# chengl7-lab/scape

Measured on AMD Instinct MI355X. Metric: UTR regions/sec (infer_pa EM to convergence), 50k UTRs x 2k reads synthetic, higher is better.
Workload: dtype f64; 1 GPU; 50k-UTR synthetic stream x 2000 reads, K=1..10 x 10 restarts; step = one resident batch of 512 UTRs per GPU; reads_per_utr=2000, k_cap=10, n_frag_max=1469, re_run_mode=False, rng_mode=per_utr, parallelism=utr-shard x1

## Files before the change

scape_amd/csrc/em_lockstep.inc:

```

#define MT_RB 1
#define MT_ROWS (64 * MT_RB)
#define MT_NC 32
#define MT_PITCH (MT_NC + 2)
#define MT_VPITCH (MT_NC + 2)
#define MT_MAXJ 64
#ifndef EM_DEPTH
#define EM_DEPTH 3
#endif
static_assert(EM_DEPTH >= 1 && EM_DEPTH <= 8, "column slots per job");
#ifndef MT_DV1
#define MT_DV1 1
#endif

#ifndef MT_DEEP
#define MT_DEEP 2
#endif
#define CNT_DONE 3
#define CNT_SLAB 4
#define CNT_EXEC (4 + 64)
#define CNT_MSTEP_TENSOR (4 + 2 * 64)
#define CNT_MSTEP_VREQ (4 + 3 * 64)
#define CNT_MSTEP_VUNI (4 + 4 * 64)
static_assert(MT_ROWS == TILE_ROWS, "tile height must match k_tile_extent / the host tables");
static_assert(MT_MAXJ <= 64, "the per-pass job setup gives one job to each lane of one wavefront");

struct EmState {
    int32_t *ia, *ib, *sia, *sib;
    double *ws, *slw;
    double *lb, *ell;
    int32_t *nlb, *status;
    unsigned long long *pend;
    int32_t *rd_k, *rd_lo, *rd_hi, *rd_m;
    int32_t *rd_n0, *rd_n1;
    double *rd_lw, *rd_sv;
    double *rd_fl;
    double *V;
    double *Vsuf;
    const int64_t *voff;
    double *pt_score;
    int32_t *pt_row;
    const int64_t *ptoff;
    int32_t *u_done;
};

__device__ __forceinline__ double d_wave_allsum(double v) {
#pragma unroll
    for (int off = 32; off > 0; off >>= 1) v += __shfl_xor(v, off, 64);
    return v;
}

#ifndef ESTEP_EXP_GROUP
#define ESTEP_EXP_GROUP 1
#endif
struct EstepNext {
    int status;
    int nlb;
    int pub_k;
    int k_next;
};

template <int CA, int CX, int NW = 1>
__device__ __forceinline__ EstepNext estep_body(
    const UtrDesc *__restrict__ descs, const DevParams &P, const double *__restrict__ cnt,
    const double *__restrict__ M, int kmax, const int32_t *__restrict__ job_utr,
    const int32_t *__restrict__ job_K, const int32_t *__restrict__ job_fixed,
    const int32_t *__restrict__ a_in, const int32_t *__restrict__ b_in,
    const double *__restrict__ ws_in, const int8_t *__restrict__ k_arr, const EmState &S,
    int32_t *__restrict__ a_out, int32_t *__restrict__ b_out, double *__restrict__ ws_out,
    double *__restrict__ bic_out, int32_t *__restrict__ nlb_out, double *__restrict__ lb_out,
    unsigned long long *__restrict__ counters, int launch, int slot, int depth, int job, int lane, int status,
    unsigned long long *s_roff, double *s_lwc, double *s_wsum ,
    const double2 *s_exptab , int wave = 0, double *s_xz = nullptr ,
    double *s_tot = nullptr ) {
    constexpr int CMAX = CA;
#ifdef ESTEP_STAMPS
    const unsigned long long st0 = __builtin_amdgcn_s_memtime();
#define ESTEP_STAMP(v) const unsigned long long v = __builtin_amdgcn_s_memtime()
#else
#define ESTEP_STAMP(v)
#endif
    const bool lead = (NW == 1) || wave == 0;
    const int nround = P.nround, B = P.B;
    const int u_job = job_utr[job];
    const int K = (CX > 0) ? CX - 1 : job_K[job], C = K + 1;
    const bool fixed = job_fixed[job] != 0;
    int32_t *ia = S.ia + (size_t)job * kmax, *ib = S.ib + (size_t)job * kmax;
    int32_t *sia = S.sia + (size_t)job * kmax, *sib = S.sib + (size_t)job * kmax;
    double *ws = S.ws + (size_t)job * (kmax + 1), *slw = S.slw + (size_t)job * (kmax + 1);
    const bool r0 = launch == 0 && slot == 0;
    const bool resolve = slot == 0 && launch > 0;
    const size_t col0 = (size_t)job * depth, col = col0 + slot;
    int pre_m[EM_DEPTH], pre_lo[EM_DEPTH], pre_hi[EM_DEPTH], pre_k[EM_DEPTH];
    int64_t pre_ptoff[EM_DEPTH];
    double pre_fl[EM_DEPTH];
    bool rdm = false;
#pragma unroll
    for (int q = 0; q < EM_DEPTH; ++q) {
        const bool on = resolve && q < depth;
        pre_m[q] = on ? S.rd_m[col0 + q] : 0;
        pre_lo[q] = on ? S.rd_lo[col0 + q] : 0;
        pre_hi[q] = on ? S.rd_hi[col0 + q] : 0;
        pre_k[q] = on ? S.rd_k[col0 + q] : 0;
        pre_ptoff[q] = on ? S.ptoff[col0 + q] : 0;
        pre_fl[q] = on ? S.rd_fl[col0 + q] : 0.0;
        rdm = rdm || pre_m[q] != 0;
    }
    const int64_t pre_voff = S.voff[col];
    const int k_lane = (lane < nround) ? (int)k_arr[(size_t)job * nround + lane] : 0;
    const double lb_prev = r0 ? SENT : S.lb[job];
    const int nlb_prev = r0 ? 0 : S.nlb[job];
    auto k_of_round = [&](int i) {
        const int ii = min(i, nround - 1);
        return (nround <= 64) ? __shfl(k_lane, ii, 64) : (int)k_arr[(size_t)job * nround + ii];
    };
    const int k_now = k_of_round(nlb_prev);
    const int k_next = __builtin_amdgcn_readfirstlane(k_of_round(nlb_prev + 1));
    double my_ws = 0.0, my_slw = 0.0;
    int my_ia = 0, my_ib = 0, my_sia = 0, my_sib = 0;
    if (lane < C) {
        my_ws = r0 ? ws_in[(size_t)job * (kmax + 1) + lane] : ws[lane];
        if (!r0) my_slw = slw[lane];
        if (lane < K) {
            my_ia = r0 ? a_in[(size_t)job * kmax + lane] : ia[lane];
            my_ib = r0 ? b_in[(size_t)job * kmax + lane] : ib[lane];
            my_sia = r0 ? my_ia : sia[lane];
            my_sib = r0 ? my_ib : sib[lane];
        }
    }
    const UtrDesc d = descs[u_job];
    double pt_best[EM_DEPTH];
    int pt_best_r[EM_DEPTH];
#pragma unroll
    for (int q = 0; q < EM_DEPTH; ++q) {
        pt_best[q] = -INFINITY;
        pt_best_r[q] = pre_lo[q];
        if (pre_m[q]) {
            const int t0 = pre_lo[q] / MT_ROWS, t1 = (pre_hi[q] - 1) / MT_ROWS;
            const double fl = pre_fl[q], ftol = (4.0 * d.Np + 16.0) * 1.1102230246251565e-16 * fabs(fl);
            for (int t = t0 + lane; t <= t1; t += 64) {
                double sc = S.pt_score[pre_ptoff[q] + t];
                const int rr = S.pt_row[pre_ptoff[q] + t];
                if (fabs(sc - fl) <= ftol) sc = fl;
                if (sc > pt_best[q]) {
                    pt_best[q] = sc;
                    pt_best_r[q] = rr;
                }
            }
        }
    }
    const int N = d.N, Np = d.Np;
    const double *Mu = M + (size_t)d.m_off;
    const double *cu = cnt + d.bin_off;
    if (r0) my_slw = d_logw(my_ws);

    if (lead && r0) {
        if (lane < C) {
            ws[lane] = my_ws;
            slw[lane] = my_slw;
            if (lane < K) {
                ia[lane] = sia[lane] = my_ia;
                ib[lane] = sib[lane] = my_ib;
            }
        }
        if (lane == 0) {
            S.lb[job] = SENT;
            S.nlb[job] = 0;
            S.ell[job] = 0.0;
        }
    }
    int upd_k[EM_DEPTH], upd_a[EM_DEPTH], upd_b[EM_DEPTH];
#pragma unroll
    for (int q = 0; q < EM_DEPTH; ++q) {
        upd_k[q] = -1;
        upd_a[q] = upd_b[q] = 0;
        if (pre_m[q]) {
            double best = pt_best[q];
            int best_r = pt_best_r[q];
#pragma unroll
            for (int off = 32; off > 0; off >>= 1) {
                const double ob = __shfl_xor(best, off, 64);
                const int orr = __shfl_xor(best_r, off, 64);
                if (ob > best || (ob == best && orr < best_r)) {
                    best = ob;
                    best_r = orr;
                }
            }
            upd_k[q] = pre_k[q];
            upd_a[q] = best_r / B;
            upd_b[q] = best_r - upd_a[q] * B;
            if (lead && lane == 0) {
                ia[upd_k[q]] = upd_a[q];
                ib[upd_k[q]] = upd_b[q];
            }
            if (lane == upd_k[q]) {
                my_ia = upd_a[q];
                my_ib = upd_b[q];
            }
        }
    }
    if (slot == 0 && lead && lane == 0 && (r0 || rdm))
        for (int q = 0; q < depth; ++q) S.rd_m[col0 + q] = 0;
    auto cur_ia = [&](int i) {
        int v = ia[i];
#pragma unroll
        for (int q = 0; q < EM_DEPTH; ++q) v = (i == upd_k[q]) ? upd_a[q] : v;
        return v;
    };
    auto cur_ib = [&](int i) {
        int v = ib[i];
#pragma unroll
        for (int q = 0; q < EM_DEPTH; ++q) v = (i == upd_k[q]) ? upd_b[q] : v;
        return v;
    };

    if (status == 1 || nlb_prev >= nround) {
        if (lead && lane == 0) {
            const int n_lb = S.nlb[job];
            bic_out[job] = d_bic(S.ell[job], K, N);
            nlb_out[job] = n_lb;
            int idx[CMAX];
            for (int i = 0; i < K; ++i) idx[i] = i;
            for (int i = 1; i < K; ++i) {
                const int v = idx[i];
                int j = i - 1;
                while (j >= 0 && cur_ia(idx[j]) > cur_ia(v)) {
                    idx[j + 1] = idx[j];
                    --j;
                }
                idx[j + 1] = v;
            }
            for (int i = 0; i < K; ++i) {
                a_out[(size_t)job * kmax + i] = cur_ia(idx[i]);
                b_out[(size_t)job * kmax + i] = cur_ib(idx[i]);
                ws_out[(size_t)job * (kmax + 1) + i] = ws[idx[i]];
            }
            ws_out[(size_t)job * (kmax + 1) + K] = ws[K];
            for (int i = K; i < kmax; ++i) {
                a_out[(size_t)job * kmax + i] = -1;
                b_out[(size_t)job * kmax + i] = -1;
                ws_out[(size_t)job * (kmax + 1) + i + 1] = 0.0;
            }
            S.status[job] = 2;
            atomicAdd(&counters[CNT_DONE], 1ull);
            if (S.u_done) atomicAdd(&S.u_done[u_job], 1);
            atomicAdd(&counters[0], (unsigned long long)n_lb);
            atomicAdd(&counters[2], (unsigned long long)n_lb * (unsigned long long)N * (unsigned long long)C);
        }
        return EstepNext{2, nlb_prev, -1, 0};
    }

    if (lead && lane == 0) atomicAdd(&counters[CNT_EXEC + (job & 63)], 1ull);
    const int k = k_now;
    const double wk_old = __shfl(my_ws, k, 64);
    const double slw_k = d_logw(wk_old);
    const int sia_k = (k < K) ? __shfl(my_ia, k, 64) : 0;
    const int sib_k = (k < K) ? __shfl(my_ib, k, 64) : 0;
    const int ia_km1 = __shfl(my_ia, max(k - 1, 0), 64), ia_kp1 = __shfl(my_ia, min(k + 1, 63), 64);
    if (lead && lane == 0) {
        slw[k] = slw_k;
        if (k < K) {
            sia[k] = sia_k;
            sib[k] = sib_k;
        }
    }
    if (lead && lane < CMAX) {
        const int c = lane;
        int sa = 0, sb = 0;
        double lw_c = 0.0;
        if (c < C) {
            if (c == k) {
                lw_c = slw_k;
                sa = sia_k;
                sb = sib_k;
            } else {
                lw_c = my_slw;
                sa = my_sia;
                sb = my_sib;
            }
        }
        s_roff[c] = (c < K) ? ((unsigned long long)sa * B + sb) * Np : 0ull;
        s_lwc[c] = (c < K) ? lw_c : lw_c + d.unif_ll;
    }
    __syncthreads();
    double *Vj = S.V + pre_voff;

    ESTEP_STAMP(st1);
    double tot_w[CMAX], t_sumk = 0.0, t_ell = 0.0, t_ent = 0.0;
    int nz_lo = 0x7fffffff, nz_hi = -1;
    bool mod = false;
    if constexpr (NW == 1) {
        for (int pass = 0; pass < 2; ++pass) {
    #pragma unroll
            for (int c = 0; c < CMAX; ++c) s_wsum[c * 64 + lane] = 0.0;
            double sumk = 0.0, ell = 0.0, ent = 0.0;
            nz_lo = 0x7fffffff;
            nz_hi = -1;
            double mcur[CMAX], ccur = 0.0;
            auto fetch = [&](int n, double (&m)[CMAX], double &cn) {
                const bool ok = n < N;
                cn = ok ? cu[n] : 0.0;
    #pragma unroll
                for (int c = 0; c < CMAX; ++c) m[c] = (ok && c < K) ? Mu[s_roff[c] + n] : 0.0;
            };
            fetch(lane, mcur, ccur);
    #pragma unroll
            for (int c = 0; c < CMAX; ++c) asm volatile("" : "+v"(mcur[c]));
            asm volatile("" : "+v"(ccur));
            for (int n = lane; n < Np; n += 64) {
                double mnext[CMAX], cnext;
                fetch(n + 64, mnext, cnext);
                double vkn = 0.0;
                if (n < N) {
                    const double cn = ccur;
                    auto lzv = [&](int c) { return (c < K) ? s_lwc[c] + mcur[c] : s_lwc[c]; };
                    double mx = 0.0;
    #pragma unroll
                    for (int c = 0; c < CMAX; ++c) {
                        if (c < C) {
                            const double v = lzv(c);
                            mx = (c == 0 || v > mx) ? v : mx;
                        }
                    }
                    double z[CMAX];
                    unsigned long long live = 0ull;
#if ESTEP_EXP_GROUP >= 2
    #pragma unroll
                    for (int c = 0; c < CMAX; c += ESTEP_EXP_GROUP) {
    #pragma unroll
                        for (int i = 0; i < ESTEP_EXP_GROUP; ++i)
                            if (c + i < CMAX) z[c + i] = 0.0;
                        if (c < C) {
                            double arg[ESTEP_EXP_GROUP];
                            bool any_live = false;
    #pragma unroll
                            for (int i = 0; i < ESTEP_EXP_GROUP; ++i) {
                                const bool in = (c + i < CMAX) && (c + i < C);
                                arg[i] = in ? (lzv((c + i < CMAX) ? c + i : c) - mx) * cn : -1000.0;
                                any_live |= arg[i] >= -746.0;
                            }
                            if (__ballot(any_live)) {
    #pragma unroll
                                for (int i = 0; i < ESTEP_EXP_GROUP; ++i)
                                    if (c + i < CMAX)
                                        if (c + i < C) {
                                            live |= 1ull << (c + i);
                                            z[c + i] = d_exp_nonpos(arg[i], s_exptab);
                                        }
                            }
                            __builtin_amdgcn_sched_barrier(0);
                        }
                    }
#else
    #pragma unroll
                    for (int c = 0; c < CMAX; ++c) {
                        z[c] = 0.0;
                        if (c < C) {
                            const double arg = (lzv(c) - mx) * cn;
                            if (__ballot(arg >= -746.0)) {
                                live |= 1ull << c;
                                z[c] = d_exp_nonpos(arg, s_exptab);
                            }
                            __builtin_amdgcn_sched_barrier(0);
                        }
                    }
#endif
                    const double s = d_np_sum<CMAX>(z, C);
                    const double rs = d_rcp_mid(s);
                    double zk = 0.0;
    #pragma unroll
                    for (int c = 0; c < CMAX; ++c) {
                        if (live & (1ull << c)) z[c] = z[c] * rs;
                        if (c == k) {
                            sumk += z[c];
                            if (mod) z[c] += 1e-8;
                            zk = z[c];
                        }
                    }
                    const double s2 = d_np_sum<CMAX>(z, C);
                    const double x2 = s2 - 1.0;
                    const double ls = d_log_pos(s), rs2 = d_rcp_mid(s2);
                    double ls2 = x2 - 0.5 * x2 * x2;
                    if (__ballot(fabs(x2) >= 1e-5)) ls2 = (fabs(x2) < 1e-5) ? ls2 : log(s2);
                    double lzk_mod = 0.0;
                    if (mod) lzk_mod = log(zk);
                    double en = 0.0;
    #pragma unroll
                    for (int c = 0; c < CMAX; ++c) {
                        if (c < C && ((live & (1ull << c)) || (mod && c == k))) {
                            const double lzc_full = lzv(c);
                            s_wsum[c * 64 + lane] += cn * z[c];
                            if (z[c] != 0.0) ell += (z[c] * cn) * lzc_full;
                            const double pk = z[c] * rs2;
                            const double lzc = (mod && c == k) ? lzk_mod : (lzc_full - mx) * cn - ls;
                            en += (pk > 0.0) ? -pk * (lzc - ls2) : 0.0;
                        }
                    }
                    ent += cn * en;
                    vkn = zk * cn;
                }
                Vj[n] = vkn;
                if (vkn != 0.0) {
                    nz_lo = min(nz_lo, n);
                    nz_hi = n;
                }
    #pragma unroll
                for (int c = 0; c < CMAX; ++c) mcur[c] = mnext[c];
                ccur = cnext;
            }
    #pragma unroll
            for (int c = 0; c < CMAX; ++c) tot_w[c] = d_wave_allsum(s_wsum[c * 64 + lane]);
            t_sumk = d_wave_allsum(sumk);
            t_ell = d_wave_allsum(ell);
            t_ent = d_wave_allsum(ent);
            if (pass == 0 && t_sumk < 1e-8) {
                mod = true;
                continue;
            }
            break;
        }
    } else {
        for (int pass = 0; pass < 2; ++pass) {
#pragma unroll
            for (int c = 0; c < CMAX; ++c)
                if ((c % NW) == wave) s_wsum[c * 64 + lane] = 0.0;
            double sumk = 0.0, ell = 0.0, ent = 0.0;
            nz_lo = 0x7fffffff;
            nz_hi = -1;
            double mcur[CMAX], ccur = 0.0;
            auto fetch = [&](int n, double (&m)[CMAX], double &cn) {
                const bool ok = n < N;
                cn = ok ? cu[n] : 0.0;
#pragma unroll
                for (int c = 0; c < CMAX; ++c) m[c] = (ok && c < K) ? Mu[s_roff[c] + n] : 0.0;
            };
            fetch(lane, mcur, ccur);
#pragma unroll
            for (int c = 0; c < CMAX; ++c) asm volatile("" : "+v"(mcur[c]));
            asm volatile("" : "+v"(ccur));
            int buf = 0;
            for (int n0 = 0; n0 < Np; n0 += 64, buf ^= 1) {
                const int n = n0 + lane;
                double mnext[CMAX], cnext;
                fetch(n + 64, mnext, cnext);
                double *xz = s_xz + (size_t)buf * (CMAX * 64);
                const double cn = ccur;
                auto lzv = [&](int c) { return (c < K) ? s_lwc[c] + mcur[c] : s_lwc[c]; };
                double mx = 0.0;
                if (n < N) {
#pragma unroll
                    for (int c = 0; c < CMAX; ++c) {
                        if (c < C) {
                            const double v = lzv(c);
                            mx = (c == 0 || v > mx) ? v : mx;
                        }
                    }
#pragma unroll
                    for (int c = 0; c < CMAX; ++c) {
                        if (c < C && (c % NW) == wave) {
                            const double arg = (lzv(c) - mx) * cn;
                            double zr = 0.0;
                            if (__ballot(arg >= -746.0)) zr = d_exp_nonpos(arg, s_exptab);
                            xz[c * 64 + lane] = zr;
                            __builtin_amdgcn_sched_barrier(0);
                        }
                    }
                }
                __syncthreads();
                double vkn = 0.0;
                if (n < N) {
                    double z[CMAX];
#pragma unroll
                    for (int c = 0; c < CMAX; ++c) z[c] = (c < C) ? xz[c * 64 + lane] : 0.0;
                    const double s = d_np_sum<CMAX>(z, C);
                    const double rs = d_rcp_mid(s);
                    double zk = 0.0;
#pragma unroll
                    for (int c = 0; c < CMAX; ++c) {
                        z[c] = z[c] * rs;
                        if (c == k) {
                            sumk += z[c];
                            if (mod) z[c] += 1e-8;
                            zk = z[c];
                        }
                    }
                    const double s2 = d_np_sum<CMAX>(z, C);
                    const double x2 = s2 - 1.0;
                    const double ls = d_log_pos(s), rs2 = d_rcp_mid(s2);
                    double ls2 = x2 - 0.5 * x2 * x2;
                    if (__ballot(fabs(x2) >= 1e-5)) ls2 = (fabs(x2) < 1e-5) ? ls2 : log(s2);
                    double lzk_mod = 0.0;
                    if (mod) lzk_mod = log(zk);
#pragma unroll
                    for (int c = 0; c < CMAX; ++c)
                        if (c < C && (c % NW) == wave) s_wsum[c * 64 + lane] += cn * z[c];
                    if (lead) {
                        double en = 0.0;
#pragma unroll
                        for (int c = 0; c < CMAX; ++c) {
                            if (c < C) {
                                const double lzc_full = lzv(c);
                                if (z[c] != 0.0) ell += (z[c] * cn) * lzc_full;
                                const double pk = z[c] * rs2;
                                const double lzc = (mod && c == k) ? lzk_mod : (lzc_full - mx) * cn - ls;
                                en += (pk > 0.0) ? -pk * (lzc - ls2) : 0.0;
                            }
                        }
                        ent += cn * en;
                        vkn = zk * cn;
                    }
                }
                if (lead && n < Np) {
                    Vj[n] = vkn;
                    if (vkn != 0.0) {
                        nz_lo = min(nz_lo, n);
                        nz_hi = n;
                    }
                }
#pragma unroll
                for (int c = 0; c < CMAX; ++c) mcur[c] = mnext[c];
                ccur = cnext;
            }
#pragma unroll
            for (int c = 0; c < CMAX; ++c) {
                if ((c % NW) == wave) {
                    const double t = d_wave_allsum(s_wsum[c * 64 + lane]);
                    if (lane == 0) s_tot[c] = t;
                }
            }
            if (lead) {
                t_sumk = d_wave_allsum(sumk);
                t_ell = d_wave_allsum(ell);
                t_ent = d_wave_allsum(ent);
                if (lane == 0) s_tot[CMAX] = (pass == 0 && t_sumk < 1e-8) ? 1.0 : 0.0;
            }
            __syncthreads();
#pragma unroll
            for (int c = 0; c < CMAX; ++c) tot_w[c] = s_tot[c];
            const bool redo = s_tot[CMAX] != 0.0;
            __syncthreads();
            if (redo) {
                mod = true;
                continue;
            }
            break;
        }
        if (!lead) return EstepNext{0, 0, -1, 0};
    }

    ESTEP_STAMP(st2);
    double sv = 0.0;
#pragma unroll
    for (int c = 0; c < CMAX; ++c)
        if (c == k) sv = tot_w[c];
    double wn[CMAX];
#pragma unroll
    for (int c = 0; c < CMAX; ++c) wn[c] = (c < C) ? tot_w[c] : 0.0;
    {
        const double s = d_np_sum<CMAX>(wn, C);
#pragma unroll
        for (int c = 0; c < CMAX; ++c) wn[c] = wn[c] / s;
        double wK = 0.0;
#pragma unroll
        for (int c = 0; c < CMAX; ++c)
            if (c == K) wK = wn[c];
        if (wK > P.max_unif_ws) {
            const double sk = d_np_sum<CMAX>(wn, K);
#pragma unroll
            for (int c = 0; c < CMAX; ++c) {
                if (c < K) wn[c] = (1 - P.max_unif_ws) * wn[c] / sk;
                if (c == K) wn[c] = P.max_unif_ws;
            }
        }
    }
    double wk_new = 0.0;
#pragma unroll
    for (int c = 0; c < CMAX; ++c) {
        if (c == k) wk_new = wn[c];
        if (c == lane && c < C) ws[c] = wn[c];
    }

#pragma unroll
    for (int off = 32; off > 0; off >>= 1) {
        nz_lo = min(nz_lo, __shfl_xor(nz_lo, off, 64));
        nz_hi = max(nz_hi, __shfl_xor(nz_hi, off, 64));
    }
    ESTEP_STAMP(st3);
    double v_total = 0.0;
    if (!fixed && k < K) {
        double *Sj = S.Vsuf + (pre_voff >> 4) + col;
        double carry = 0.0;
        for (int nb = ((Np - 1) >> 6) << 6; nb >= 0; nb -= 8 * 64) {
            double vv[8];
#pragma unroll
            for (int q = 0; q < 8; ++q) {
                const int n = nb - 64 * q + lane;
                vv[q] = (n >= 0 && n < Np) ? Vj[n] : 0.0;
            }
#pragma unroll
            for (int off = 1; off < 64; off <<= 1) {
#pragma unroll
                for (int q = 0; q < 8; ++q) {
                    const double t = __shfl_down(vv[q], off, 64);
                    if (lane + off < 64) vv[q] += t;
                }
            }
#pragma unroll
            for (int q = 0; q < 8; ++q) {
                const int n0 = nb - 64 * q;
                if (n0 >= 0) {
                    const int n = n0 + lane;
                    if ((lane & 15) == 0 && n < Np) Sj[n >> 4] = carry + vv[q];
                    carry += __shfl(vv[q], 0, 64);
                }
            }
        }
        if (lane == 0) Sj[Np >> 4] = 0.0;
        v_total = carry;
    }
    ESTEP_STAMP(st4);
    const double lb_new = t_ell + t_ent;
    const int status_new = (fabs(lb_new - lb_prev) < fabs(1e-6 * lb_prev)) ? 1 : 0;
    const bool has_m = (!fixed && k < K);
    if (lane == 0) {
        const int n_lb = nlb_prev;
        lb_out[(size_t)job * nround + n_lb] = lb_new;
        S.nlb[job] = n_lb + 1;
        S.ell[job] = t_ell;
        S.lb[job] = lb_new;
        S.status[job] = status_new;
        S.rd_m[col] = has_m ? 1 : 0;
        if (has_m) {
            const int lo = (k == 0) ? 0 : ia_km1;
            const int hi = (k == K - 1) ? d.T - 1 : ia_kp1;
            S.rd_k[col] = k;
            S.rd_lo[col] = lo * B;
            S.rd_hi[col] = (hi + 1) * B;
            S.rd_lw[col] = d_logw(wk_new);
            S.rd_sv[col] = sv;
            S.rd_fl[col] = d_logw(wk_new) * sv + SENT * v_total;
            S.rd_n0[col] = (nz_hi >= 0) ? nz_lo : 0;
            S.rd_n1[col] = (nz_hi >= 0) ? nz_hi + 1 : 0;
            atomicAdd(&counters[CNT_SLAB + (job & 63)], (unsigned long long)(hi + 1 - lo) * B * (unsigned long long)N);
        }
    }
#ifdef ESTEP_STAMPS
    if (NW == 1 && lane == 0) {
        const unsigned long long st5 = __builtin_amdgcn_s_memtime();
        unsigned long long *sp = counters + 4 + 5 * 64;
        atomicAdd(&sp[0], st1 - st0);
        atomicAdd(&sp[1], st2 - st1);
        atomicAdd(&sp[2], st3 - st2);
        atomicAdd(&sp[3], st4 - st3);
        atomicAdd(&sp[4], st5 - st4);
        atomicAdd(&sp[7], 1ull);
    }
#endif
#undef ESTEP_STAMP
    return EstepNext{status_new, nlb_prev + 1, has_m ? k : -1, k_next};
}

#define ESTEP_ARGS(ROUND, STATUS) descs, P, cnt, M, kmax, job_utr, job_K, job_fixed, a_in, b_in, ws_in, k_arr, S, a_out, \
                   b_out, ws_out, bic_out, nlb_out, lb_out, counters, ROUND, slot, depth, job, lane, STATUS, s_roff, s_lwc, s_wsum, s_exptab
#define ESTEP_CASE(C, ROUND, STATUS) \
    case C: nx = estep_body<C, C, ESTEP_NW>(ESTEP_ARGS(ROUND, STATUS) ESTEP_EXTRA); break;
#define ESTEP_DISPATCH(CM, ROUND, STATUS)                                                         \
    do {                                                                                          \
        if constexpr (CM <= 16) {                                                                 \
            const int c_exact = job_K[job] + 1;                                                   \
            if constexpr (CM >= 16) {                                                             \
                if (c_exact > 12) {                                                               \
                    switch (c_exact) {                                                            \
                        ESTEP_CASE(13, ROUND, STATUS) ESTEP_CASE(14, ROUND, STATUS)               \
                        ESTEP_CASE(15, ROUND, STATUS)                                             \
                        default: nx = estep_body<16, 16, ESTEP_NW>(ESTEP_ARGS(ROUND, STATUS) ESTEP_EXTRA); break;            \
                    }                                                                             \
                    break;                                                                        \
                }                                                                                 \
            }                                                                                     \
            if constexpr (CM >= 12) {                                                             \
                if (c_exact > 8) {                                                                \
                    switch (c_exact) {                                                            \
                        ESTEP_CASE(9, ROUND, STATUS) ESTEP_CASE(10, ROUND, STATUS)                \
                        ESTEP_CASE(11, ROUND, STATUS)                                             \
                        default: nx = estep_body<12, 12, ESTEP_NW>(ESTEP_ARGS(ROUND, STATUS) ESTEP_EXTRA); break;            \
                    }                                                                             \
                    break;                                                                        \
                }                                                                                 \
            }                                                                                     \
            if constexpr (CM >= 8) {                                                              \
                if (c_exact > 4) {                                                                \
                    switch (c_exact) {                                                            \
                        ESTEP_CASE(5, ROUND, STATUS) ESTEP_CASE(6, ROUND, STATUS)                 \
                        ESTEP_CASE(7, ROUND, STATUS)                                              \
                        default: nx = estep_body<8, 8, ESTEP_NW>(ESTEP_ARGS(ROUND, STATUS) ESTEP_EXTRA); break;              \
                    }                                                                             \
                    break;                                                                        \
                }                                                                                 \
            }                                                                                     \
            switch (c_exact) {                                                                    \
                ESTEP_CASE(1, ROUND, STATUS) ESTEP_CASE(2, ROUND, STATUS) ESTEP_CASE(3, ROUND, STATUS) \
                default: nx = estep_body<4, 4, ESTEP_NW>(ESTEP_ARGS(ROUND, STATUS) ESTEP_EXTRA); break;                      \
            }                                                                                     \
        } else {                                                                                  \
            nx = estep_body<CM, 0, ESTEP_NW>(ESTEP_ARGS(ROUND, STATUS) ESTEP_EXTRA);                                       \
        }                                                                                         \
    } while (0)

__host__ __device__ inline bool em_run_ahead_stops(int status, int nlb, int nround, int k_next, unsigned long long pend) {
    return status != 0 || nlb >= nround || (pend & (7ull << k_next)) != 0ull;
}
__host__ inline int em_slots_needed(int max_k_live, int depth) {
    return std::min(depth, max_k_live <= 2 ? 1 : max_k_live == 3 ? 2 : depth);
}
__host__ inline bool em_shrink_due(long long listed, long long live, int pct) {
    return live > 0 && live < listed && live * 100 <= listed * pct;
}
__host__ __device__ inline int em_shrink_pos(int base, const int *wave_cnt, int wave, unsigned long long mask, int lane) {
    int off = base;
    for (int w = 0; w < wave; ++w) off += wave_cnt[w];
    unsigned long long below = mask & ((1ull << lane) - 1ull);
    int n = 0;
    for (; below; below &= below - 1) ++n;
    return off + n;
}

#define EM_SHRINK_THREADS 1024
#ifndef EM_SHRINK_AT
#define EM_SHRINK_AT 50
#endif
__global__ __launch_bounds__(EM_SHRINK_THREADS) void k_em_shrink(int32_t *elist, int n_list, const int32_t *__restrict__ status,
                                                                 const int32_t *__restrict__ job_K, const int32_t *__restrict__ job_fixed,
                                                                 int32_t *active, int n_active, const int32_t *__restrict__ u_done,
                                                                 const int64_t *__restrict__ ujob_off, int depth, int32_t *__restrict__ out) {
    __shared__ int s_cnt[EM_SHRINK_THREADS / 64];
    __shared__ int s_k;
    const int tid = threadIdx.x, lane = tid & 63, wave = tid >> 6;
    if (tid == 0) s_k = 0;
    int k_live = 0;
    auto compact = [&](int32_t *list, int n, auto keep) {
        int base = 0;
        for (int i0 = 0; i0 < n; i0 += EM_SHRINK_THREADS) {
            const int i = i0 + tid;
            int32_t v = 0;
            bool kp = false;
            if (i < n) {
                v = list[i];
                kp = keep(v);
            }
            const unsigned long long mask = __ballot(kp);
            if (lane == 0) s_cnt[wave] = __popcll(mask);
            __syncthreads();
            if (kp) list[em_shrink_pos(base, s_cnt, wave, mask, lane)] = v;
            for (int w = 0; w < EM_SHRINK_THREADS / 64; ++w) base += s_cnt[w];
            __syncthreads();
        }
        return base;
    };
    const int jobs = compact(elist, n_list, [&](int32_t j) {
        const bool live = status[j] != 2;
        if (live && job_fixed[j] == 0) k_live = max(k_live, job_K[j]);
        return live;
    });
    const int utrs = compact(active, n_active, [&](int32_t u) { return (int64_t)u_done[u] * depth < ujob_off[u + 1] - ujob_off[u]; });
    if (k_live) atomicMax(&s_k, k_live);
    __syncthreads();
// ... 402 lines not shown
```

scape_amd/csrc/scape_hip.hip:

```cpp
#include <hip/hip_runtime.h>

#include <algorithm>
#include <atomic>
#include <cmath>
#include <cstdint>
#include <cstdio>
#include <cstdlib>
#include <cstring>
#include <memory>
#include <string>
#include <type_traits>
#include <chrono>
#include <utility>
#include <vector>

#include "scape_hip.h"

#define SENT SCAPE_SENT
#define PI_REF 3.141592653589793
#define PITCH 16
#define TILE_ROWS 64

static thread_local std::string g_err;
static int fail(const std::string &msg) {
    g_err = msg;
    return 1;
}
#define HIPCHK(expr)                                                                         \
    do {                                                                                     \
        hipError_t e_ = (expr);                                                              \
        if (e_ != hipSuccess)                                                                \
            return fail(std::string(#expr) + ": " + hipGetErrorString(e_) + " (" + __FILE__ + \
                        ":" + std::to_string(__LINE__) + ")");                               \
    } while (0)

struct UtrDesc {
    int64_t bin_off;
    int64_t theta_off;
    int64_t at_off;
    int64_t m_off;
    int64_t log_off;
    int64_t tile_off;
    int64_t mlog_off;
    int32_t c_lo, c_hi;
    int32_t N, Np, T, n_log;
    double unif_ll, L, min_theta;
};

struct DevParams {
    double mu_f, sigma_f, max_unif_ws;
    int32_t B, S, nround, pad;
    double betas[SCAPE_MAX_BETA];
    double s_dis[SCAPE_MAX_S];
    double pmf_s[SCAPE_MAX_S];
    double inv_s[SCAPE_MAX_S];
};

__device__ __forceinline__ double d_log_pos(double x) {
#pragma clang fp contract(off)
    const double ln2_hi = 6.93147180369123816490e-01, ln2_lo = 1.90821492927058770002e-10,
                 Lg1 = 6.666666666666735130e-01, Lg2 = 3.999999999940941908e-01, Lg3 = 2.857142874366239149e-01,
                 Lg4 = 2.222219843214978396e-01, Lg5 = 1.818357216161805012e-01, Lg6 = 1.531383769920937332e-01,
                 Lg7 = 1.479819860511658591e-01;
    double m = __builtin_amdgcn_frexp_mant(x);
    int e = __builtin_amdgcn_frexp_exp(x);
    const bool lo = m < 0.70710678118654752440;
    m = lo ? m * 2.0 : m;
    e = lo ? e - 1 : e;
    const double f = m - 1.0, d = 2.0 + f;
    double r = __builtin_amdgcn_rcp(d);
    r = __builtin_fma(__builtin_fma(-d, r, 1.0), r, r);
    r = __builtin_fma(__builtin_fma(-d, r, 1.0), r, r);
    double s = f * r;
    s = __builtin_fma(__builtin_fma(-d, s, f), r, s);
    const double dk = (double)e, z = s * s, w = z * z;
    const double t1 = w * __builtin_fma(w, __builtin_fma(w, Lg6, Lg4), Lg2);
    const double t2 = z * __builtin_fma(w, __builtin_fma(w, __builtin_fma(w, Lg7, Lg5), Lg3), Lg1);
    const double R = t2 + t1;
    const double hfsq = 0.5 * f * f;
    const double inner = __builtin_fma(s, hfsq + R, dk * ln2_lo);
    return dk * ln2_hi - ((hfsq - inner) - f);
}

#include "exp_table.inc"
__device__ __forceinline__ void d_load_exptab(double2 *tab , int tid, int nthreads) {
    for (int i = tid; i < 128; i += nthreads) tab[i] = g_exp_tab[i];
}
__device__ __forceinline__ double d_exp_nonpos(double x, const double2 *tab) {
#pragma clang fp contract(off)
    x = fmax(x, -750.0);
    const double n = __builtin_rint(x * EXP_INV_L);
    double r = __builtin_fma(n, -EXP_L_HI, x);
    r = __builtin_fma(n, -EXP_L_LO, r);
    const int ni = (int)n;
    const double2 t = tab[ni & 127];
    const double r2 = r * r;
    const double q = __builtin_fma(r, __builtin_fma(r, __builtin_fma(r, 1.0 / 120, 1.0 / 24), 1.0 / 6), 0.5);
    const double p = __builtin_fma(r2, q, r);
    return ldexp(t.x + __builtin_fma(t.x, p, t.y), ni >> 7);
}

__device__ __forceinline__ double d_rcp_mid(double x) {
#pragma clang fp contract(off)
    double r = __builtin_amdgcn_rcp(x);
    r = __builtin_fma(__builtin_fma(-x, r, 1.0), r, r);
    r = __builtin_fma(__builtin_fma(-x, r, 1.0), r, r);
    return r;
}

__device__ __forceinline__ double d_logw(double w) { return (w <= 0.0) ? SENT : log(w); }

__device__ __forceinline__ double d_bic(double ell, int K, int N) {
#pragma clang fp contract(off)
    const double penalty = (double)(3 * K + 1) * log((double)N);
    return -2.0 * ell + penalty;
}
__device__ __forceinline__ double d_logpdf_normal(double x, double mu, double sigma) {
    double z = (x - mu) / sigma;
    return -0.5 * (z * z) - log(sigma) - 0.5 * log(2 * PI_REF);
}
__device__ __forceinline__ double d_pdf_normal(double x, double mu, double sigma) {
    double z = (x - mu) / sigma;
    return exp(-0.5 * (z * z)) / sqrt(2 * PI_REF) / sigma;
}

__device__ __forceinline__ double d_pdf_normal_t(double x, double mu, double sigma, const double2 *tab) {
    double z = (x - mu) / sigma;
    return d_exp_nonpos(-0.5 * (z * z), tab) / sqrt(2 * PI_REF) / sigma;
}

__device__ __forceinline__ double d_point_pa(double x, double l, double pa, double th, double sigma_f) {
    double u = th - x;
    double ll_l = (l <= u) ? -log(u) : SENT;
    return ll_l + d_logpdf_normal(pa - th, 0.0, sigma_f);
}
__device__ __forceinline__ double d_point_r_unknown(double x, double l, double th, const double *s,
                                                    const double *pmf, const double *inv_s, int S, double mu_f,
                                                    double sigma_f, double *a, const double2 *tab) {
    double u = th - x;
    double v = 0.0;
    if (l <= u) {
        const double lk = 1 / u, inv_sigma = 1 / sigma_f, inv_norm = 1 / sqrt(2 * PI_REF);
        for (int j = 0; j < S; ++j) {
            const double z = (x - (th + s[j] - mu_f)) * inv_sigma;
            const double pdf = d_exp_nonpos(-0.5 * (z * z), tab) * inv_norm * inv_sigma;
            v += inv_s[j] * pdf * lk * pmf[j];
        }
    }
    if (v < 1e-300) v = 0.0;
    *a = (v <= 0.0) ? SENT : d_log_pos(v);
    return v;
}
__device__ __forceinline__ double d_point_r_known(double x, double l, double r, double th,
                                                  const double *s, const double *pmf, int S,
                                                  double mu_f, double sigma_f) {
    double u = th - x;
    double ll_l = (l <= u) ? -log(u) : SENT;
    double tmpn = 0.0, mx = 0.0;
    for (int j = 0; j < S; ++j) {
        double t;
        if (s[j] < r) {
            t = SENT;
        } else {
            tmpn += pmf[j];
            double lrs = (r <= s[j]) ? -log(s[j]) : SENT;
            t = lrs + d_logpdf_normal(x, th + s[j] - mu_f, sigma_f) + ll_l + log(pmf[j]);
        }
        if (j == 0 || t > mx) mx = t;
    }
    double sum = 0.0;
    for (int j = 0; j < S; ++j) {
        double t;
        if (s[j] < r) {
            t = SENT;
        } else {
            double lrs = (r <= s[j]) ? -log(s[j]) : SENT;
            t = lrs + d_logpdf_normal(x, th + s[j] - mu_f, sigma_f) + ll_l + log(pmf[j]);
        }
        sum += exp(t - mx);
    }
    return log(sum) + mx - log(tmpn);
}

template <int CMAX>
__device__ __forceinline__ double d_np_sum(const double (&a)[CMAX], int C) {
    if (C < 8) {
        double r = 0.0;
#pragma unroll
        for (int i = 0; i < (CMAX < 7 ? CMAX : 7); ++i)
            if (i < C) r += a[i];
        return r;
    }
    if constexpr (CMAX >= 8) {
        double r[8];
#pragma unroll
        for (int j = 0; j < 8; ++j) r[j] = a[j];
        const int lim = C - (C % 8);
#pragma unroll
        for (int i = 8; i + 8 <= CMAX; i += 8)
            if (i < lim) {
#pragma unroll
                for (int j = 0; j < 8; ++j) r[j] += a[i + j];
            }
        double res = ((r[0] + r[1]) + (r[2] + r[3])) + ((r[4] + r[5]) + (r[6] + r[7]));
#pragma unroll
        for (int i = 8; i < CMAX; ++i)
            if (i >= lim && i < C) res += a[i];
        return res;
    }
    return 0.0;
}

__global__ void k_op_pa(const double *x, const double *l, const double *pa, int n, double theta,
                        double sigma_f, double *out) {
    int i = blockIdx.x * blockDim.x + threadIdx.x;
    if (i < n) out[i] = d_point_pa(x[i], l[i], pa[i], theta, sigma_f);
}
__global__ void k_op_r_known(const double *x, const double *l, const double *r, int n, DevParams P,
                             double theta, double *out) {
    int i = blockIdx.x * blockDim.x + threadIdx.x;
    if (i < n) out[i] = d_point_r_known(x[i], l[i], r[i], theta, P.s_dis, P.pmf_s, P.S, P.mu_f, P.sigma_f);
}
__global__ void k_op_r_unknown(const double *x, const double *l, int n, DevParams P, double theta,
                               double *out) {
    __shared__ double2 s_exptab[128];
    d_load_exptab(s_exptab, threadIdx.x, blockDim.x);
    __syncthreads();
    int i = blockIdx.x * blockDim.x + threadIdx.x;
    if (i < n) {
        double a;
        d_point_r_unknown(x[i], l[i], theta, P.s_dis, P.pmf_s, P.inv_s, P.S, P.mu_f, P.sigma_f, &a, s_exptab);
        out[i] = a;
    }
}

#define PA_TT 8
__global__ __launch_bounds__(256) void k_phase_a(const UtrDesc *__restrict__ descs, DevParams P,
                                                 const double *__restrict__ x,
                                                 const double *__restrict__ l,
                                                 const double *__restrict__ r,
                                                 const double *__restrict__ pa,
                                                 const double *__restrict__ theta,
                                                 double *__restrict__ AT, double *__restrict__ V) {
    __shared__ double2 s_exptab[128];
    d_load_exptab(s_exptab, threadIdx.x, blockDim.x);
    __syncthreads();
    const UtrDesc d = descs[blockIdx.z];
    const int t0 = blockIdx.y * PA_TT, t1 = min(d.T, t0 + PA_TT);
    const int n = blockIdx.x * blockDim.x + threadIdx.x;
    if (t0 >= d.T || n >= d.Np) return;
// ... 1292 lines not shown
```

Baseline: 3508 UTRs/s.

## Micro-optimize E-step inner loop: uniform k dispatch, held poly constants, DPP scan

Bundles several instruction-level changes in the E-step hot loop. K, nlb and k are made wave-uniform via readfirstlane/readlane, and the per-component k selection becomes a compile-time switch. The two-pass mod loop becomes a templated lambda, so the common non-mod pass carries no mod branches. Log/exp polynomial constants are pinned in SGPR/VGPR registers instead of being rematerialized, conditional adds become fma, and the V prefix scan uses DPP row shifts plus readlane instead of shuffles. The main risk is small changes in floating-point rounding, since fma contraction and removing the pk>0 and z!=0 guards change summation order, and higher register pressure.

Measured after the change: 3703 UTRs/s (median of 6 runs). +5.6%, better.

```diff
diff --git a/scape_amd/csrc/em_lockstep.inc b/scape_amd/csrc/em_lockstep.inc
--- a/scape_amd/csrc/em_lockstep.inc
+++ b/scape_amd/csrc/em_lockstep.inc
@@ -53,6 +53,35 @@
 #ifndef ESTEP_EXP_GROUP
 #define ESTEP_EXP_GROUP 1
 #endif
+template <int CMAX, class F>
+__device__ __forceinline__ void d_at_uniform(int k, F &&f) {
+#define AT_CASE(i)                                                 \
+    case i:                                                        \
+        if constexpr ((i) < CMAX) f(std::integral_constant<int, (i)>{}); \
+        break;
+#define AT_CASE8(b) AT_CASE(b) AT_CASE(b + 1) AT_CASE(b + 2) AT_CASE(b + 3) AT_CASE(b + 4) AT_CASE(b + 5) AT_CASE(b + 6) AT_CASE(b + 7)
+    switch (k) {
+        AT_CASE8(0) AT_CASE8(8) AT_CASE8(16) AT_CASE8(24) AT_CASE8(32) AT_CASE8(40) AT_CASE8(48) AT_CASE8(56)
+        default: break;
+    }
+#undef AT_CASE8
+#undef AT_CASE
+}
+__device__ __forceinline__ double d_en_add(bool first, double en, double pk, double d) {
+#pragma clang fp contract(off)
+    if (first) return __builtin_fma(-pk, d, 0.0);
+    const double t = -pk * d;
+    return en + t;
+}
+template <int N>
+__device__ __forceinline__ double d_row_shl(double v) {
+    const int lo = __builtin_amdgcn_update_dpp(0, __double2loint(v), 0x100 + N, 0xf, 0xf, true);
+    const int hi = __builtin_amdgcn_update_dpp(0, __double2hiint(v), 0x100 + N, 0xf, 0xf, true);
+    return __hiloint2double(hi, lo);
+}
+__device__ __forceinline__ double d_lane_value(double v, int l) {
+    return __hiloint2double(__builtin_amdgcn_readlane(__double2hiint(v), l), __builtin_amdgcn_readlane(__double2loint(v), l));
+}
 struct EstepNext {
     int status;
     int nlb;
@@ -83,7 +112,7 @@
     const bool lead = (NW == 1) || wave == 0;
     const int nround = P.nround, B = P.B;
     const int u_job = job_utr[job];
-    const int K = (CX > 0) ? CX - 1 : job_K[job], C = K + 1;
+    const int K = (CX > 0) ? CX - 1 : __builtin_amdgcn_readfirstlane(job_K[job]), C = K + 1;
     const bool fixed = job_fixed[job] != 0;
     int32_t *ia = S.ia + (size_t)job * kmax, *ib = S.ib + (size_t)job * kmax;
     int32_t *sia = S.sia + (size_t)job * kmax, *sib = S.sib + (size_t)job * kmax;
@@ -109,12 +138,12 @@
     const int64_t pre_voff = S.voff[col];
     const int k_lane = (lane < nround) ? (int)k_arr[(size_t)job * nround + lane] : 0;
     const double lb_prev = r0 ? SENT : S.lb[job];
-    const int nlb_prev = r0 ? 0 : S.nlb[job];
+    const int nlb_prev = r0 ? 0 : __builtin_amdgcn_readfirstlane(S.nlb[job]);
     auto k_of_round = [&](int i) {
         const int ii = min(i, nround - 1);
         return (nround <= 64) ? __shfl(k_lane, ii, 64) : (int)k_arr[(size_t)job * nround + ii];
     };
-    const int k_now = k_of_round(nlb_prev);
+    const int k_now = __builtin_amdgcn_readfirstlane(k_of_round(nlb_prev));
     const int k_next = __builtin_amdgcn_readfirstlane(k_of_round(nlb_prev + 1));
     double my_ws = 0.0, my_slw = 0.0;
     int my_ia = 0, my_ib = 0, my_sia = 0, my_sib = 0;
@@ -254,9 +283,9 @@
     const int k = k_now;
     const double wk_old = __shfl(my_ws, k, 64);
     const double slw_k = d_logw(wk_old);
-    const int sia_k = (k < K) ? __shfl(my_ia, k, 64) : 0;
-    const int sib_k = (k < K) ? __shfl(my_ib, k, 64) : 0;
-    const int ia_km1 = __shfl(my_ia, max(k - 1, 0), 64), ia_kp1 = __shfl(my_ia, min(k + 1, 63), 64);
+    const int sia_k = (k < K) ? __builtin_amdgcn_readlane(my_ia, k) : 0;
+    const int sib_k = (k < K) ? __builtin_amdgcn_readlane(my_ib, k) : 0;
+    const int ia_km1 = __builtin_amdgcn_readlane(my_ia, max(k - 1, 0)), ia_kp1 = __builtin_amdgcn_readlane(my_ia, min(k + 1, 63));
     if (lead && lane == 0) {
         slw[k] = slw_k;
         if (k < K) {
@@ -288,28 +317,23 @@
     ESTEP_STAMP(st1);
     double tot_w[CMAX], t_sumk = 0.0, t_ell = 0.0, t_ent = 0.0;
     int nz_lo = 0x7fffffff, nz_hi = -1;
-    bool mod = false;
+    const ExpPoly exp_poly = d_exp_poly_held();
+    const LogPoly log_poly = d_log_poly_held();
     if constexpr (NW == 1) {
-        for (int pass = 0; pass < 2; ++pass) {
+        auto run_pass = [&](auto mod_c) {
+            constexpr bool mod = decltype(mod_c)::value;
     #pragma unroll
             for (int c = 0; c < CMAX; ++c) s_wsum[c * 64 + lane] = 0.0;
             double sumk = 0.0, ell = 0.0, ent = 0.0;
             nz_lo = 0x7fffffff;
             nz_hi = -1;
-            double mcur[CMAX], ccur = 0.0;
             auto fetch = [&](int n, double (&m)[CMAX], double &cn) {
                 const bool ok = n < N;
                 cn = ok ? cu[n] : 0.0;
     #pragma unroll
                 for (int c = 0; c < CMAX; ++c) m[c] = (ok && c < K) ? Mu[s_roff[c] + n] : 0.0;
             };
-            fetch(lane, mcur, ccur);
-    #pragma unroll
-            for (int c = 0; c < CMAX; ++c) asm volatile("" : "+v"(mcur[c]));
-            asm volatile("" : "+v"(ccur));
-            for (int n = lane; n < Np; n += 64) {
-                double mnext[CMAX], cnext;
-                fetch(n + 64, mnext, cnext);
+            auto bin_step = [&](int n, const double (&mcur)[CMAX], double ccur) {
                 double vkn = 0.0;
                 if (n < N) {
                     const double cn = ccur;
@@ -319,7 +343,7 @@
                     for (int c = 0; c < CMAX; ++c) {
                         if (c < C) {
                             const double v = lzv(c);
-                            mx = (c == 0 || v > mx) ? v : mx;
+                            mx = (c == 0) ? v : fmax(mx, v);
                         }
                     }
                     double z[CMAX];
@@ -345,7 +369,7 @@
                                     if (c + i < CMAX)
                                         if (c + i < C) {
                                             live |= 1ull << (c + i);
-                                            z[c + i] = d_exp_nonpos(arg[i], s_exptab);
+                                            z[c + i] = d_exp_nonpos(arg[i], s_exptab, exp_poly);
                                         }
                             }
                             __builtin_amdgcn_sched_barrier(0);
@@ -359,7 +383,7 @@
                             const double arg = (lzv(c) - mx) * cn;
                             if (__ballot(arg >= -746.0)) {
                                 live |= 1ull << c;
-                                z[c] = d_exp_nonpos(arg, s_exptab);
+                                z[c] = d_exp_nonpos(arg, s_exptab, exp_poly);
                             }
                             __builtin_amdgcn_sched_barrier(0);
                         }
@@ -369,31 +393,31 @@
                     const double rs = d_rcp_mid(s);
                     double zk = 0.0;
     #pragma unroll
-                    for (int c = 0; c < CMAX; ++c) {
-                        if (live & (1ull << c)) z[c] = z[c] * rs;
-                        if (c == k) {
-                            sumk += z[c];
-                            if (mod) z[c] += 1e-8;
-                            zk = z[c];
-                        }
-                    }
+                    for (int c = 0; c < CMAX; ++c) z[c] = z[c] * rs;
+                    d_at_uniform<CMAX>(k, [&](auto ck) {
+                        constexpr int c = decltype(ck)::value;
+                        zk = z[c];
+                        if (mod) z[c] += 1e-8;
+                    });
+                    sumk += zk;
+                    if (mod) zk += 1e-8;
                     const double s2 = d_np_sum<CMAX>(z, C);
                     const double x2 = s2 - 1.0;
-                    const double ls = d_log_pos(s), rs2 = d_rcp_mid(s2);
+                    const double ls = d_log_pos(s, log_poly), rs2 = d_rcp_mid(s2);
                     double ls2 = x2 - 0.5 * x2 * x2;
                     if (__ballot(fabs(x2) >= 1e-5)) ls2 = (fabs(x2) < 1e-5) ? ls2 : log(s2);
                     double lzk_mod = 0.0;
-                    if (mod) lzk_mod = log(zk);
+                    if constexpr (mod) lzk_mod = log(zk);
                     double en = 0.0;
     #pragma unroll
                     for (int c = 0; c < CMAX; ++c) {
                         if (c < C && ((live & (1ull << c)) || (mod && c == k))) {
                             const double lzc_full = lzv(c);
-                            s_wsum[c * 64 + lane] += cn * z[c];
-                            if (z[c] != 0.0) ell += (z[c] * cn) * lzc_full;
+                            s_wsum[c * 64 + lane] = __builtin_fma(cn, z[c], s_wsum[c * 64 + lane]);
+                            ell = __builtin_fma(z[c] * cn, lzc_full, ell);
                             const double pk = z[c] * rs2;
                             const double lzc = (mod && c == k) ? lzk_mod : (lzc_full - mx) * cn - ls;
-                            en += (pk > 0.0) ? -pk * (lzc - ls2) : 0.0;
+                            en = d_en_add(c == 0, en, pk, lzc - ls2);
                         }
                     }
                     ent += cn * en;
@@ -404,6 +428,15 @@
                     nz_lo = min(nz_lo, n);
                     nz_hi = n;
                 }
+            };
+            double mcur[CMAX], mnext[CMAX], ccur = 0.0, cnext = 0.0;
+            fetch(lane, mcur, ccur);
+    #pragma unroll
+            for (int c = 0; c < CMAX; ++c) asm volatile("" : "+v"(mcur[c]));
+            asm volatile("" : "+v"(ccur));
+            for (int n = lane; n < Np; n += 64) {
+                fetch(n + 64, mnext, cnext);
+                bin_step(n, mcur, ccur);
     #pragma unroll
                 for (int c = 0; c < CMAX; ++c) mcur[c] = mnext[c];
                 ccur = cnext;
@@ -413,14 +446,12 @@
             t_sumk = d_wave_allsum(sumk);
             t_ell = d_wave_allsum(ell);
             t_ent = d_wave_allsum(ent);
-            if (pass == 0 && t_sumk < 1e-8) {
-                mod = true;
-                continue;
-            }
-            break;
-        }
+            return !mod && t_sumk < 1e-8;
+        };
+        if (run_pass(std::false_type{})) run_pass(std::true_type{});
     } else {
-        for (int pass = 0; pass < 2; ++pass) {
+        auto run_pass = [&](auto mod_c) {
+            constexpr bool mod = decltype(mod_c)::value;
 #pragma unroll
             for (int c = 0; c < CMAX; ++c)
                 if ((c % NW) == wave) s_wsum[c * 64 + lane] = 0.0;
@@ -452,7 +483,7 @@
                     for (int c = 0; c < CMAX; ++c) {
                         if (c < C) {
                             const double v = lzv(c);
-                            mx = (c == 0 || v > mx) ? v : mx;
+                            mx = (c == 0) ? v : fmax(mx, v);
                         }
                     }
 #pragma unroll
@@ -460,7 +491,7 @@
                         if (c < C && (c % NW) == wave) {
                             const double arg = (lzv(c) - mx) * cn;
                             double zr = 0.0;
-                            if (__ballot(arg >= -746.0)) zr = d_exp_nonpos(arg, s_exptab);
+                            if (__ballot(arg >= -746.0)) zr = d_exp_nonpos(arg, s_exptab, exp_poly);
                             xz[c * 64 + lane] = zr;
                             __builtin_amdgcn_sched_barrier(0);
                         }
@@ -476,34 +507,34 @@
                     const double rs = d_rcp_mid(s);
                     double zk = 0.0;
 #pragma unroll
-                    for (int c = 0; c < CMAX; ++c) {
-                        z[c] = z[c] * rs;
-                        if (c == k) {
-                            sumk += z[c];
-                            if (mod) z[c] += 1e-8;
-                            zk = z[c];
-                        }
-                    }
+                    for (int c = 0; c < CMAX; ++c) z[c] = z[c] * rs;
+                    d_at_uniform<CMAX>(k, [&](auto ck) {
+                        constexpr int c = decltype(ck)::value;
+                        zk = z[c];
+                        if (mod) z[c] += 1e-8;
+                    });
+                    sumk += zk;
+                    if (mod) zk += 1e-8;
                     const double s2 = d_np_sum<CMAX>(z, C);
                     const double x2 = s2 - 1.0;
-                    const double ls = d_log_pos(s), rs2 = d_rcp_mid(s2);
+                    const double ls = d_log_pos(s, log_poly), rs2 = d_rcp_mid(s2);
                     double ls2 = x2 - 0.5 * x2 * x2;
                     if (__ballot(fabs(x2) >= 1e-5)) ls2 = (fabs(x2) < 1e-5) ? ls2 : log(s2);
                     double lzk_mod = 0.0;
-                    if (mod) lzk_mod = log(zk);
+                    if constexpr (mod) lzk_mod = log(zk);
 #pragma unroll
                     for (int c = 0; c < CMAX; ++c)
-                        if (c < C && (c % NW) == wave) s_wsum[c * 64 + lane] += cn * z[c];
+                        if (c < C && (c % NW) == wave) s_wsum[c * 64 + lane] = __builtin_fma(cn, z[c], s_wsum[c * 64 + lane]);
                     if (lead) {
                         double en = 0.0;
 #pragma unroll
                         for (int c = 0; c < CMAX; ++c) {
                             if (c < C) {
                                 const double lzc_full = lzv(c);
-                                if (z[c] != 0.0) ell += (z[c] * cn) * lzc_full;
+                                ell = __builtin_fma(z[c] * cn, lzc_full, ell);
                                 const double pk = z[c] * rs2;
                                 const double lzc = (mod && c == k) ? lzk_mod : (lzc_full - mx) * cn - ls;
-                                en += (pk > 0.0) ? -pk * (lzc - ls2) : 0.0;
+                                en = d_en_add(c == 0, en, pk, lzc - ls2);
                             }
                         }
                         ent += cn * en;
@@ -532,19 +563,16 @@
                 t_sumk = d_wave_allsum(sumk);
                 t_ell = d_wave_allsum(ell);
                 t_ent = d_wave_allsum(ent);
-                if (lane == 0) s_tot[CMAX] = (pass == 0 && t_sumk < 1e-8) ? 1.0 : 0.0;
+                if (lane == 0) s_tot[CMAX] = (!mod && t_sumk < 1e-8) ? 1.0 : 0.0;
             }
             __syncthreads();
 #pragma unroll
             for (int c = 0; c < CMAX; ++c) tot_w[c] = s_tot[c];
             const bool redo = s_tot[CMAX] != 0.0;
             __syncthreads();
-            if (redo) {
-                mod = true;
-                continue;
-            }
-            break;
-        }
+            return redo;
+        };
+        if (run_pass(std::false_type{})) run_pass(std::true_type{});
         if (!lead) return EstepNext{0, 0, -1, 0};
     }
 
@@ -598,20 +626,23 @@
                 vv[q] = (n >= 0 && n < Np) ? Vj[n] : 0.0;
             }
 #pragma unroll
-            for (int off = 1; off < 64; off <<= 1) {
-#pragma unroll
-                for (int q = 0; q < 8; ++q) {
-                    const double t = __shfl_down(vv[q], off, 64);
-                    if (lane + off < 64) vv[q] += t;
-                }
+            for (int q = 0; q < 8; ++q) {
+                vv[q] += d_row_shl<1>(vv[q]);
+                vv[q] += d_row_shl<2>(vv[q]);
+                vv[q] += d_row_shl<4>(vv[q]);
+                vv[q] += d_row_shl<8>(vv[q]);
             }
 #pragma unroll
             for (int q = 0; q < 8; ++q) {
                 const int n0 = nb - 64 * q;
                 if (n0 >= 0) {
                     const int n = n0 + lane;
-                    if ((lane & 15) == 0 && n < Np) Sj[n >> 4] = carry + vv[q];
-                    carry += __shfl(vv[q], 0, 64);
+                    const double T0 = d_lane_value(vv[q], 0), T1 = d_lane_value(vv[q], 16), T2 = d_lane_value(vv[q], 32),
+                                 T3 = d_lane_value(vv[q], 48);
+                    const double S32 = T2 + T3, S16 = (T1 + T2) + T3, S0 = (T0 + T1) + S32;
+                    const double mine = (lane < 16) ? S0 : (lane < 32) ? S16 : (lane < 48) ? S32 : T3;
+                    if ((lane & 15) == 0 && n < Np) Sj[n >> 4] = carry + mine;
+                    carry += S0;
                 }
             }
         }
diff --git a/scape_amd/csrc/scape_hip.hip b/scape_amd/csrc/scape_hip.hip
--- a/scape_amd/csrc/scape_hip.hip
+++ b/scape_amd/csrc/scape_hip.hip
@@ -56,12 +56,31 @@
     double inv_s[SCAPE_MAX_S];
 };
 
-__device__ __forceinline__ double d_log_pos(double x) {
+struct LogPoly {
+    double Lg1, Lg2, Lg3, Lg4, Lg5, Lg6, Lg7;
+};
+struct ExpPoly {
+    double c5, c4, c3;
+};
+#define D_LOG_POLY LogPoly{6.666666666666735130e-01, 3.999999999940941908e-01, 2.857142874366239149e-01, 2.222219843214978396e-01, \
+                           1.818357216161805012e-01, 1.531383769920937332e-01, 1.479819860511658591e-01}
+#define D_EXP_POLY ExpPoly{1.0 / 120, 1.0 / 24, 1.0 / 6}
+__device__ __forceinline__ LogPoly d_log_poly_held() {
+    LogPoly k = D_LOG_POLY;
+    asm volatile("" : "+s"(k.Lg1), "+s"(k.Lg2), "+s"(k.Lg3), "+s"(k.Lg6), "+s"(k.Lg7));
+    asm volatile("" : "+v"(k.Lg4), "+v"(k.Lg5));
+    return k;
+}
+__device__ __forceinline__ ExpPoly d_exp_poly_held() {
+    ExpPoly k = D_EXP_POLY;
+    asm volatile("" : "+s"(k.c5), "+s"(k.c3));
+    asm volatile("" : "+v"(k.c4));
+    return k;
+}
+__device__ __forceinline__ double d_log_pos(double x, const LogPoly &k = D_LOG_POLY) {
 #pragma clang fp contract(off)
     const double ln2_hi = 6.93147180369123816490e-01, ln2_lo = 1.90821492927058770002e-10,
-                 Lg1 = 6.666666666666735130e-01, Lg2 = 3.999999999940941908e-01, Lg3 = 2.857142874366239149e-01,
-                 Lg4 = 2.222219843214978396e-01, Lg5 = 1.818357216161805012e-01, Lg6 = 1.531383769920937332e-01,
-                 Lg7 = 1.479819860511658591e-01;
+                 Lg1 = k.Lg1, Lg2 = k.Lg2, Lg3 = k.Lg3, Lg4 = k.Lg4, Lg5 = k.Lg5, Lg6 = k.Lg6, Lg7 = k.Lg7;
     double m = __builtin_amdgcn_frexp_mant(x);
     int e = __builtin_amdgcn_frexp_exp(x);
     const bool lo = m < 0.70710678118654752440;
@@ -86,7 +105,7 @@
 __device__ __forceinline__ void d_load_exptab(double2 *tab , int tid, int nthreads) {
     for (int i = tid; i < 128; i += nthreads) tab[i] = g_exp_tab[i];
 }
-__device__ __forceinline__ double d_exp_nonpos(double x, const double2 *tab) {
+__device__ __forceinline__ double d_exp_nonpos(double x, const double2 *tab, const ExpPoly &k = D_EXP_POLY) {
 #pragma clang fp contract(off)
     x = fmax(x, -750.0);
     const double n = __builtin_rint(x * EXP_INV_L);
@@ -95,7 +114,7 @@
     const int ni = (int)n;
     const double2 t = tab[ni & 127];
     const double r2 = r * r;
-    const double q = __builtin_fma(r, __builtin_fma(r, __builtin_fma(r, 1.0 / 120, 1.0 / 24), 1.0 / 6), 0.5);
+    const double q = __builtin_fma(r, __builtin_fma(r, __builtin_fma(r, k.c5, k.c4), k.c3), 0.5);
     const double p = __builtin_fma(r2, q, r);
     return ldexp(t.x + __builtin_fma(t.x, p, t.y), ni >> 7);
 }
```
